# ArturKKK/graphcast-lite

Measured on AMD Instinct MI355X. Metric: training samples/sec (6h windows) + achieved HBM GB/s on mesh GCNConv, higher is better.
Workload: dtype f32

## Files before the change

graphcast-lite_amd/csrc/linear.hip:

```cpp
#include "common.h"
#include "mfma_io.h"
#include "x3.h"

namespace {

using namespace gcl::mfma_io;

#include "gemm_tile.h"

#define gcl_lin_sync() ((abl & 8) != 0)

constexpr int lin_min_waves(int NS, int KT) { return (NS <= 2 && KT <= 64) ? 3 : (NS <= 2 && KT <= 128) ? 2 : 1; }
constexpr bool lin_zpre(int NS, int EPI) { return EPI == 1 && NS >= 4; }

template <int NS, int EPI, int KT, bool VEC>
__global__ __launch_bounds__(256, lin_min_waves(NS, KT)) void linear_mfma_kernel(const float* __restrict__ X, int64_t ldx,
                                                          const float* __restrict__ in_slope,
                                                          const float* __restrict__ W, int32_t ldw, int32_t trans,
                                                          const float* __restrict__ bias, float* __restrict__ Y,
                                                          int64_t ldy, int64_t rows, int32_t K, int32_t N,
                                                          const float* __restrict__ Z, int64_t ldz,
                                                          const float* __restrict__ z_slope,
                                                          double* __restrict__ slope_part, int32_t akind,
                                                          int32_t abl) {
// ... 1152 lines not shown
  do {                                                                                                            \
    auto kern = gemm_tile_kernel<EPI, T_, MI_>;                                                                   \
    GCL_ENSURE_DYN_LDS(kern, gcl::kLdsBytes);                                                                     \
    hipLaunchKernelGGL(kern, dim3(g.grid), dim3(256), gt_lds(MI_), st, X, ldx, akind, slope, W, ldw, bias, Y, ldy, \
                       rows, K, N, Z, ldz, add, ldadd, slope_part, g.nt, g.total, g.per_xcd);                     \
  } while (0)
  if (trans) {
    if (g.mi == 1) GCL_GT(true, 1);
    else GCL_GT(true, 2);
  } else {
    if (g.mi == 1) GCL_GT(false, 1);
    else GCL_GT(false, 2);
  }
#undef GCL_GT
  GCL_CHECK_LAUNCH();
  if (nparts) *nparts = (int)g.grid;
  return GCL_OK;
}

}

extern "C" size_t gcl_colsum_ws_bytes(int64_t, int32_t);
extern "C" int gcl_colsum(const float*, int64_t, int64_t, int32_t, float*, int32_t, void*, size_t, gcl_stream_t);

static int check_act(const char* who, int act, const float* slope) {
  GCL_CHECK_ARG(act == GCL_ACT_NONE || act == GCL_ACT_PRELU || act == GCL_ACT_SILU, "%s: unknown activation %d", who, act);
  GCL_CHECK_ARG(act != GCL_ACT_PRELU || slope, "%s: GCL_ACT_PRELU needs the slope pointer", who);
  return GCL_OK;
}

extern "C" int gcl_dense_fwd(const float* x, int64_t ldx, int32_t act, const float* slope, const float* W, int64_t ldw,
                             const float* bias, const float* addend, int64_t ldadd, float* y, int64_t ldy,
                             int64_t rows, int32_t Fin, int32_t Fout, gcl_stream_t stream) {
  GCL_CHECK_ARG(x && W && y, "dense_fwd: null argument");
  GCL_CHECK_ARG(rows >= 0 && Fin >= 1 && Fout >= 1 && ldx >= Fin && ldy >= Fout && ldw >= Fin && (!addend || ldadd >= Fout),
                "dense_fwd: bad shape rows=%lld ldx=%lld ldy=%lld ldw=%lld", (long long)rows, (long long)ldx,
                (long long)ldy, (long long)ldw);
  if (int rc = check_act("dense_fwd", act, slope)) return rc;
  const bool vec_x = (Fin % 4 == 0) && (ldx % 4 == 0) && gcl::aligned16(x);
  if (!addend && ldw == Fin && !use_valu() && gcl::x3_linear_fwd_applicable(x, ldx, y, ldy, Fin, Fout, act))
    return gcl::x3_linear_fwd(x, ldx, act, act == GCL_ACT_PRELU ? slope : nullptr, W, bias, y, ldy, rows, Fin, Fout,
                              (hipStream_t)stream);
  if (!addend && ldw == Fin && (use_valu() || panel_fits(Fin, Fout, vec_x, false, (ldw % 4 == 0) && gcl::aligned16(W))))
    return launch_linear<EPI_BIAS>(x, ldx, act == GCL_ACT_PRELU ? slope : nullptr, W, Fin, 0, bias, y, ldy, rows, Fin,
                                   Fout, nullptr, 0, nullptr, nullptr, nullptr, (hipStream_t)stream, act);
  return launch_gemm<EPI_BIAS>(x, ldx, act, act == GCL_ACT_PRELU ? slope : nullptr, W, ldw, 0, bias, y, ldy, rows, Fin,
                               Fout, nullptr, 0, addend, ldadd, nullptr, nullptr, (hipStream_t)stream);
}

extern "C" int gcl_linear_fwd(const float* x, int64_t ldx, const float* in_slope, const float* W, const float* bias,
                              float* y, int64_t ldy, int64_t rows, int32_t Fin, int32_t Fout, gcl_stream_t stream) {
  return gcl_dense_fwd(x, ldx, in_slope ? GCL_ACT_PRELU : GCL_ACT_NONE, in_slope, W, Fin, bias, nullptr, 0, y, ldy, rows,
                       Fin, Fout, stream);
}

static size_t slope_parts_cap(int64_t rows, int32_t Fin) {
  const int64_t g = (int64_t)gt_geom(rows, Fin).grid;
  return (size_t)(g > 4096 ? g : 4096);
}

extern "C" size_t gcl_linear_bwd_ws_bytes(int64_t rows, int32_t Fin, int32_t Fout) {
  size_t nc = (size_t)(Fin + 31) / 32;
  if (nc > 4) nc = 4;
  const size_t FinP = nc * 32;
  size_t no = (size_t)(Fout + 31) / 32;
  no = no <= 2 ? no : no <= 4 ? 4 : 8;
  const size_t FoutP = no * 32;
  const size_t dw = (size_t)kDwBlocks * FoutP * (FinP + 1) * sizeof(float);
  const size_t sl = slope_parts_cap(rows, Fin) * sizeof(double);
  return dw + sl;
}

extern "C" int gcl_dense_bwd_dx(const float* dy, int64_t lddy, const float* W, int64_t ldw, const float* z, int64_t ldz,
                                int32_t act, const float* slope, float* d_slope, const float* addend, int64_t ldadd,
                                float* dx, int64_t lddx, int64_t rows, int32_t Fin, int32_t Fout, void* ws,
                                size_t ws_bytes, gcl_stream_t stream) {
  GCL_CHECK_ARG(dy && W && dx, "dense_bwd_dx: null argument");
  GCL_CHECK_ARG(lddy >= Fout && lddx >= Fin && ldw >= Fin && (!addend || ldadd >= Fin), "dense_bwd_dx: leading dimension too small");
  if (int rc = check_act("dense_bwd_dx", act, slope)) return rc;
  GCL_CHECK_ARG(act == GCL_ACT_NONE || (z && ldz >= Fin), "dense_bwd_dx: activation given without its pre-activation z");
  hipStream_t st = (hipStream_t)stream;
  const float* sl = act == GCL_ACT_PRELU ? slope : nullptr;
  double* slope_part = nullptr;
  if (sl && d_slope) {
    GCL_CHECK_ARG(ws && ws_bytes >= slope_parts_cap(rows, Fin) * sizeof(double) && gcl::aligned16(ws), "dense_bwd_dx: workspace too small");
    slope_part = (double*)ws;
  }
  int nparts = 0, rc;
  const float* zz = act == GCL_ACT_NONE ? nullptr : z;
  const bool vec_x = (Fout % 4 == 0) && (lddy % 4 == 0) && gcl::aligned16(dy);
  if (!addend && ldw == Fin && (use_valu() || panel_fits(Fout, Fin, vec_x, true, (ldw % 4 == 0) && gcl::aligned16(W))))
    rc = launch_linear<EPI_DX>(dy, lddy, nullptr, W, Fin, 1, nullptr, dx, lddx, rows, Fout, Fin, zz, ldz, sl, slope_part,
                               &nparts, st, act);
  else {
    const size_t off = (slope_parts_cap(rows, Fin) * sizeof(double) + 255) & ~(size_t)255;
    const size_t need = off + (size_t)Fin * Fout * sizeof(float);
    if (ws && ws_bytes >= need && gcl::aligned16(ws) && Fout % 4 == 0 && rows >= 4096) {
      float* Wt = reinterpret_cast<float*>(static_cast<char*>(ws) + off);
      hipLaunchKernelGGL(transpose_kernel, dim3((unsigned)gcl::cdiv(Fin, 32), (unsigned)gcl::cdiv(Fout, 32)), dim3(256), 0,
                         st, W, ldw, Wt, Fout, Fin);
      rc = launch_gemm<EPI_DX>(dy, lddy, act, sl, Wt, Fout, 0, nullptr, dx, lddx, rows, Fout, Fin, zz, ldz, addend,
                               ldadd, slope_part, &nparts, st);
    } else {
      rc = launch_gemm<EPI_DX>(dy, lddy, act, sl, W, ldw, 1, nullptr, dx, lddx, rows, Fout, Fin, zz, ldz, addend, ldadd,
                               slope_part, &nparts, st);
    }
// ... 351 lines not shown
```

graphcast-lite_amd/csrc/linear_x3.hip:

```cpp
#include "mfma_io.h"
#include "x3.h"

namespace {

typedef unsigned int u32x2 __attribute__((ext_vector_type(2)));

#ifndef GCL_X3_ST_AUX
#define GCL_X3_ST_AUX 2
#endif
__device__ __forceinline__ float4 ld_stream(const float4* p) {
#ifndef GCL_X3_LD_PLAIN
  typedef float lv4f __attribute__((ext_vector_type(4)));
  const lv4f v = __builtin_nontemporal_load(reinterpret_cast<const lv4f*>(p));
  return make_float4(v.x, v.y, v.z, v.w);
#else
  return *p;
#endif
}
using namespace gcl::mfma_io;
using namespace gcl::x3;

constexpr int kRowB = 144;
constexpr int kImgB = 32 * kRowB;
constexpr int kTileB = 3 * kImgB;
// ... 149 lines not shown
        const bf16x8 am = *reinterpret_cast<const bf16x8*>(ap + kImgB);
#pragma unroll
        for (int c = 0; c < NS; ++c) acc[c] = mfma_mid(acc[c], ah, am, wf[c][s][0], wf[c][s][1]);
      }
#pragma unroll
      for (int s = 0; s < NKS; ++s) {
        const bf16x8 ah = *reinterpret_cast<const bf16x8*>(Aw + fo + s * 32);
#pragma unroll
        for (int c = 0; c < NS; ++c) acc[c] = mfma_hi(acc[c], ah, wf[c][s][0]);
      }
    }

#ifdef GCL_STAMPS
    asm volatile("" ::"v"(acc[0][0]));
#endif
    X3_STAMP(4);
    const int64_t r0 = t * 128 + wave * 32;
    const int64_t nr64 = rows - r0;
    const int nr = nr64 < 0 ? 0 : (nr64 < 32 ? (int)nr64 : 32);
    constexpr int OS = NS * 32, LPO = OS / 4, RPP = 64 / LPO;
    float* Ot = reinterpret_cast<float*>(Aw);
#pragma unroll
    for (int s = 0; s < NS; ++s)
#pragma unroll
      for (int r = 0; r < 16; ++r) Ot[d_row(r, lane) * OS + s * 32 + (lane & 31)] = acc[s][r];
    const __amdgpu_buffer_rsrc_t ry = make_rsrc(Y + r0 * ldy, (nr > 0 && !(abl & 1)) ? ((int64_t)(nr - 1) * ldy + N) * 4 : 0);
    const int orow = lane / LPO, ocol = (lane % LPO) * 4;
#pragma unroll
    for (int p = 0; p < 32 / RPP; ++p) {
      const int i = p * RPP + orow;
      float4 v = *reinterpret_cast<const float4*>(Ot + i * OS + ocol);
      v.x += bq.x; v.y += bq.y; v.z += bq.z; v.w += bq.w;
      buf_st4<GCL_X3_ST_AUX>(ry, (ocol < N) ? (unsigned)((i * ldy + ocol) * 4) : kOOB, v);
    }
    X3_STAMP(5);
  }
#ifdef GCL_STAMPS
  if (lane == 0 && blockIdx.x < 1024)
    for (int i = 0; i < 8; ++i) x3_stamps[(blockIdx.x * 4 + wave) * 8 + i] = stamp_acc[i];
#endif
}

constexpr int kBRowB = 128;
constexpr int kImg64B = 64 * kBRowB;
__device__ __forceinline__ int swz(int r) { return (((r >> 1) & 1) << 2) | (((r >> 3) & 1) << 1) | ((r >> 2) & 1); }
__device__ __forceinline__ int sw_off(int r, int b) { return r * kBRowB + ((((b >> 4) ^ swz(r)) << 4) | (b & 15)); }

typedef short s16x4 __attribute__((ext_vector_type(4)));
__device__ __forceinline__ bf16x8 tr_frag(const unsigned char* base, int o0, int o1) {
  typedef __attribute__((address_space(3))) s16x4 lds_s16x4;
  const s16x4 a = __builtin_amdgcn_ds_read_tr16_b64_v4i16((lds_s16x4*)(base + o0));
  const s16x4 b = __builtin_amdgcn_ds_read_tr16_b64_v4i16((lds_s16x4*)(base + o1));
  return __builtin_shufflevector(a, b, 0, 1, 2, 3, 4, 5, 6, 7);
}

template <int NO>
__global__ __launch_bounds__(256, 2) void linear_x3_bwd_kernel(
    const float* __restrict__ dY, int64_t lddy, const float* __restrict__ W, const float* __restrict__ P,
    int64_t ldp, const float* __restrict__ in_slope, float* __restrict__ dX, int64_t lddx, int64_t rows, int32_t Fin,
    int32_t Fout, float* __restrict__ part_dw, float* __restrict__ part_db, float* __restrict__ part_cs,
    double* __restrict__ part_slope) {
  constexpr int FoP = NO * 32, FiP = 64, NKO = NO * 2, NT = NO * 2;
  extern __shared__ __align__(16) unsigned char smem8[];
  unsigned char* Yimg = smem8;
  unsigned char* Pimg = smem8 + 3 * kImg64B;
  float* Stg = reinterpret_cast<float*>(smem8 + 6 * kImg64B);
  const int tid = threadIdx.x, lane = tid & 63, wave = __builtin_amdgcn_readfirstlane(tid >> 6);
  const int li = lane & 31, h = lane >> 5;
  const int rg = wave & 1, sg = wave >> 1;
  const int so = wave % NO, sc = wave / NO;
  const bool has_tile = wave < NT;

  bf16x8 wtf[NKO][3];
  {
    float2 wv[8];
#pragma unroll
    for (int i = 0; i < 8; ++i) {
      const int idx = i * 256 + tid;
      const int c = idx & 63, o = (idx >> 6) * 2;
      wv[i].x = (c < Fin && o < Fout) ? W[(int64_t)o * Fin + c] : 0.f;
      wv[i].y = (c < Fin && o + 1 < Fout) ? W[(int64_t)(o + 1) * Fin + c] : 0.f;
    }
#pragma unroll
    for (int i = 0; i < 8; ++i) {
      const int idx = i * 256 + tid;
      const int c = idx & 63, o = (idx >> 6) * 2;
      const Pk3 p = split2(wv[i].x, wv[i].y);
      unsigned char* d = Yimg + sw_off(c, o * 2);
      *reinterpret_cast<unsigned*>(d) = p.h;
      *reinterpret_cast<unsigned*>(d + kImg64B) = p.m;
      *reinterpret_cast<unsigned*>(d + 2 * kImg64B) = p.l;
    }
    __syncthreads();
#pragma unroll
    for (int s = 0; s < NKO; ++s)
#pragma unroll
      for (int p = 0; p < 3; ++p)
        wtf[s][p] = *reinterpret_cast<const bf16x8*>(Yimg + p * kImg64B + sw_off(32 * sg + li, (16 * s + 8 * h) * 2));
    __syncthreads();
  }

  const bool act = in_slope != nullptr;
  const float slope = act ? *in_slope : 1.f;
  const int64_t ntiles = (rows + 63) / 64;

  const int rsub = lane >> 4, csub = lane & 15;
// ... 172 lines not shown
  return 0;
#endif
  static const int v = gcl::env_int("GCL_ABLATE", 0);
  return v;
}

}

#ifdef GCL_STAMPS
extern "C" int gcl_debug_read_stamps_x3(unsigned long long* host_out, int count) {
  GCL_CHECK_HIP(hipDeviceSynchronize());
  GCL_CHECK_HIP(hipMemcpyFromSymbol(host_out, HIP_SYMBOL(x3_stamps), sizeof(unsigned long long) * count));
  return GCL_OK;
}
#endif

namespace gcl {

bool x3_linear_fwd_applicable(const float* x, int64_t ldx, const float* y, int64_t ldy, int K, int N, int akind) {
  if (!env_int("GCL_X3", 1)) return false;
  if (K < 1 || K > 64 || N < 4 || N > 64 || (N & 3)) return false;
  if ((ldx & 3) || (ldy & 3) || !aligned16(x) || !aligned16(y)) return false;
  if (ldx * 4 * 35 >= ((int64_t)1 << 31) || ldy * 4 * 35 >= ((int64_t)1 << 31)) return false;
  return akind == kActNone || akind == kActPrelu || akind == kActSilu;
}

int x3_linear_fwd(const float* x, int64_t ldx, int akind, const float* slope, const float* W, const float* bias,
                  float* y, int64_t ldy, int64_t rows, int K, int N, hipStream_t st) {
  if (rows == 0) return GCL_OK;
  const int64_t ntiles = cdiv(rows, 128);
  const int grid = (int)(ntiles < 2 * kNumCU ? ntiles : 2 * kNumCU);
  const size_t lds = 4 * (size_t)kTileB;
#define GCL_X3F3(NS_, SILU_, NKS_)                                                                                \
  hipLaunchKernelGGL((linear_x3_fwd_kernel<NS_, SILU_, NKS_>), dim3(grid), dim3(256), lds, st, x, ldx, slope, akind, \
                     W, bias, y, ldy, rows, K, N, x3_ablate())
#define GCL_X3F(NS_, SILU_)           \
  do {                                \
    if (K <= 32) GCL_X3F3(NS_, SILU_, 2); \
    else GCL_X3F3(NS_, SILU_, 4);     \
  } while (0)
  if (akind == kActSilu) {
    if (N > 32) GCL_X3F(2, true);
    else GCL_X3F(1, true);
  } else {
    if (N > 32) GCL_X3F(2, false);
    else GCL_X3F(1, false);
  }
#undef GCL_X3F3
#undef GCL_X3F
  GCL_CHECK_LAUNCH();
  return GCL_OK;
}

bool x3_linear_bwd_applicable(const float* dy, int64_t lddy, const float* x, int64_t ldx, const float* dx, int64_t lddx,
                              int Fin, int Fout) {
  if (!env_int("GCL_X3", 1)) return false;
  if (Fin < 33 || Fin > 64 || (Fin & 3) || Fout < 1 || Fout > 64) return false;
  if (lddy < ((Fout + 3) & ~3) || (lddy & 3) || (ldx & 3) || (lddx & 3) || lddx < Fin) return false;
  if (!aligned16(dy) || !aligned16(x) || !aligned16(dx)) return false;
  return lddx * 4 * 70 < ((int64_t)1 << 31);
}

int x3_linear_bwd_blocks(int64_t rows) {
  const int64_t ntiles = cdiv(rows, 64);
  return (int)(ntiles < 2 * kNumCU ? ntiles : 2 * kNumCU);
}

int x3_linear_bwd(const float* dy, int64_t lddy, const float* W, const float* x, int64_t ldx, const float* in_slope,
                  float* dx, int64_t lddx, int64_t rows, int Fin, int Fout, float* part_dw, float* part_db,
                  float* part_cs, double* part_slope, hipStream_t st) {
  const int grid = x3_linear_bwd_blocks(rows);
  const size_t lds = 6 * (size_t)kImg64B + 64 * 64 * sizeof(float);
#define GCL_X3B(NO_)                                                                                              \
  do {                                                                                                            \
    auto kern = linear_x3_bwd_kernel<NO_>;                                                                        \
    GCL_ENSURE_DYN_LDS(kern, gcl::kLdsBytes);                                                                     \
    hipLaunchKernelGGL(kern, dim3(grid), dim3(256), lds, st, dy, lddy, W, x, ldx, in_slope, dx, lddx, rows, Fin, Fout, \
                       part_dw, part_db, part_cs, part_slope);                                                    \
  } while (0)
  if (Fout > 32) GCL_X3B(2);
  else GCL_X3B(1);
#undef GCL_X3B
  GCL_CHECK_LAUNCH();
  return GCL_OK;
}

}
```

graphcast-lite_amd/csrc/x3.h:

```cpp
#pragma once
#include "common.h"

namespace gcl {

bool x3_linear_fwd_applicable(const float* x, int64_t ldx, const float* y, int64_t ldy, int K, int N, int akind);
int x3_linear_fwd(const float* x, int64_t ldx, int akind, const float* slope, const float* W, const float* bias,
                  float* y, int64_t ldy, int64_t rows, int K, int N, hipStream_t st);

bool x3_linear_bwd_applicable(const float* dy, int64_t lddy, const float* x, int64_t ldx, const float* dx, int64_t lddx,
                              int Fin, int Fout);
int x3_linear_bwd_blocks(int64_t rows);
int x3_linear_bwd(const float* dy, int64_t lddy, const float* W, const float* x, int64_t ldx, const float* in_slope,
                  float* dx, int64_t lddx, int64_t rows, int Fin, int Fout, float* part_dw, float* part_db,
                  float* part_cs, double* part_slope, hipStream_t st);

}

#ifdef __HIPCC__
#include "mfma_io.h"

namespace gcl {
namespace x3 {

using mfma_io::f32x16;
typedef short bf16x8 __attribute__((ext_vector_type(8)));
typedef __bf16 bf16x2_t __attribute__((ext_vector_type(2)));
typedef float f32x2_t __attribute__((ext_vector_type(2)));

__device__ __forceinline__ unsigned pk_bf16(float a, float b) {
  return __builtin_bit_cast(unsigned, __builtin_convertvector(f32x2_t{a, b}, bf16x2_t));
}
struct Pk3 {
  unsigned h, m, l;
};
__device__ __forceinline__ Pk3 split2(float a, float b) {
  Pk3 p;
  p.h = pk_bf16(a, b);
  float ra = a - __uint_as_float(p.h << 16), rb = b - __uint_as_float(p.h & 0xffff0000u);
  p.m = pk_bf16(ra, rb);
  ra -= __uint_as_float(p.m << 16);
  rb -= __uint_as_float(p.m & 0xffff0000u);
  p.l = pk_bf16(ra, rb);
  return p;
}

__device__ __forceinline__ f32x16 mfma_lo(f32x16 acc, bf16x8 ah, bf16x8 am, bf16x8 al, bf16x8 bh, bf16x8 bm, bf16x8 bl) {
  acc = __builtin_amdgcn_mfma_f32_32x32x16_bf16(al, bh, acc, 0, 0, 0);
  acc = __builtin_amdgcn_mfma_f32_32x32x16_bf16(ah, bl, acc, 0, 0, 0);
  acc = __builtin_amdgcn_mfma_f32_32x32x16_bf16(am, bm, acc, 0, 0, 0);
  return acc;
}
__device__ __forceinline__ f32x16 mfma_mid(f32x16 acc, bf16x8 ah, bf16x8 am, bf16x8 bh, bf16x8 bm) {
  acc = __builtin_amdgcn_mfma_f32_32x32x16_bf16(am, bh, acc, 0, 0, 0);
  acc = __builtin_amdgcn_mfma_f32_32x32x16_bf16(ah, bm, acc, 0, 0, 0);
  return acc;
}
__device__ __forceinline__ f32x16 mfma_hi(f32x16 acc, bf16x8 ah, bf16x8 bh) {
  return __builtin_amdgcn_mfma_f32_32x32x16_bf16(ah, bh, acc, 0, 0, 0);
}

// ... 4 lines not shown
```

graphcast-lite_amd/functional.py:

```python
from typing import List, Optional

import os

import torch

from . import hip


def _grad_slot(p: Optional[torch.Tensor], needs: bool):
    if p is None or not needs:
        return None, False, True
    if p.grad is not None:
        return p.grad, True, True
    return torch.zeros_like(p), False, False


class _Grads:

    def __init__(self, params: List[Optional[torch.Tensor]], needs: List[bool]):
        self.dst, self.acc, self.ret_none = [], [], []
        for p, nd in zip(params, needs):
            d, a, r = _grad_slot(p, nd)
            self.dst.append(d)
            self.acc.append(a)
            self.ret_none.append(r)

    def out(self):
        return tuple(None if r else d for d, r in zip(self.dst, self.ret_none))


_ZERO = {}


def _token(like: torch.Tensor, shape):
    z = _ZERO.get(like.device)
    if z is None:
        if like.is_cuda and torch.cuda.is_current_stream_capturing():
            return like.new_zeros(()).expand(shape)
        with torch.inference_mode(False):
            z = _ZERO[like.device] = torch.zeros((), dtype=torch.float32, device=like.device)
    return z.expand(shape)


def _flat3(x: torch.Tensor):
    if x.dim() == 2:
        x = x.unsqueeze(0)
    if not x.is_contiguous():
        x = x.contiguous()
    return x


class MLPFn(torch.autograd.Function):
    @staticmethod
    def forward(ctx, x, owner, has_ln: bool, eps: float, *params):
        L = (len(params) - (2 if has_ln else 0) + 1) // 3
        shape = x.shape
        x2 = hip.rows2d(x.detach())
        zs = []
        cur, slope = x2, None
        for k in range(L):
            W, b = params[3 * k], params[3 * k + 1]
            z = hip.linear_fwd(cur, W.detach(), b.detach(), slope)
            zs.append(z)
            cur = z
            slope = params[3 * k + 2].detach() if k < L - 1 else None
        stats = None
        out = cur
        if has_ln:
            out, stats = hip.layernorm_fwd(cur, params[-2].detach(), params[-1].detach(), eps)
        ctx.owner, ctx.has_ln, ctx.L = owner, has_ln, L
        ctx.x2, ctx.zs, ctx.stats = x2, zs, stats
        ctx.params = params
        return out.view(shape[:-1] + (out.shape[-1],))

    @staticmethod
    def backward(ctx, dy):
        params, L = ctx.params, ctx.L
        needs = list(ctx.needs_input_grad[4:])
        G = _Grads(list(params), needs)
        dy2 = hip.rows2d(dy)
        zs = ctx.zs
        if ctx.has_ln:
            gi, bi = len(params) - 2, len(params) - 1
            dgam = G.dst[gi] if G.dst[gi] is not None else torch.zeros_like(params[gi])
            dbet = G.dst[bi] if G.dst[bi] is not None else torch.zeros_like(params[bi])
            dz = hip.layernorm_bwd(dy2, zs[-1], params[gi].detach(), ctx.stats, dgam, dbet, G.acc[gi] and G.acc[bi])
        else:
            dz = dy2
        dx = None
        for k in range(L - 1, -1, -1):
            W = params[3 * k].detach()
            inp = ctx.x2 if k == 0 else zs[k - 1]
            slope = None if k == 0 else params[3 * k - 1].detach()
            wi, bi = 3 * k, 3 * k + 1
            dW = G.dst[wi] if G.dst[wi] is not None else torch.zeros_like(params[wi])
            db = G.dst[bi]
            if k > 0:
                dz = hip.linear_bwd_all(dz, W, inp, slope, G.dst[3 * k - 1], dW, db, None, G.acc[wi], acc_db=G.acc[bi])
            elif ctx.needs_input_grad[0]:
                dx = hip.linear_bwd_all(dz, W, inp, None, None, dW, db, None, G.acc[wi], acc_db=G.acc[bi],
                                        act=hip.ACT_NONE)
            elif db is not None and G.acc[bi] != G.acc[wi]:
                hip.linear_bwd_dw(dz, inp, None, dW, None, G.acc[wi])
                hip.colsum(dz, db, G.acc[bi])
            else:
                hip.linear_bwd_dw(dz, inp, None, dW, db, G.acc[wi])
        if dx is not None:
            dx = dx.view(dy.shape[:-1] + (dx.shape[-1],))
        return (dx, None, None, None) + G.out()


_LN_COLSUM = os.environ.get("GCL_NO_LN_COLSUM", "0") in ("0", "")
_ROWS_OUT = os.environ.get("GCL_NO_ROWS_OUT", "0") in ("0", "")


def _row_skip() -> bool:
    return os.environ.get("GCL_NO_ROW_SKIP", "0") in ("0", "")

# ... 801 lines not shown
```

graphcast-lite_amd/hip.py:

```python
import ctypes as C
import os
from typing import Optional

import torch

_HERE = os.path.dirname(os.path.abspath(__file__))
LIB_PATH = os.environ.get("GCL_LIB") or os.path.join(_HERE, "libgcl_hip.so")

GRAPH_GCN, GRAPH_GAT, GRAPH_MEAN = 0, 1, 2

_lib = None

_i32, _i64, _f32, _vp, _sz = C.c_int32, C.c_int64, C.c_float, C.c_void_p, C.c_size_t

_SIGNATURES = {
    "gcl_version": (C.c_int, []),
    "gcl_last_error": (C.c_char_p, []),
    "gcl_graph_count_edges": (C.c_int, [_vp, _i64, _i32, _i32, C.POINTER(_i64)]),
    "gcl_graph_build_host": (C.c_int, [_vp, _i64, _i32, _i32] + [_vp] * 8),
    "gcl_graph_create": (C.c_int, [_vp, _i64, _i32, _i32, C.POINTER(_vp)]),
    "gcl_graph_destroy": (None, [_vp]),
    "gcl_graph_num_nodes": (_i32, [_vp]),
    "gcl_graph_num_edges": (_i64, [_vp]),
    "gcl_graph_max_in_degree": (_i32, [_vp]),
    "gcl_graph_export_edges": (C.c_int, [_vp, _vp]),
    "gcl_graph_eperm_device": (_vp, [_vp]),
    "gcl_graph_halo_info": (C.c_int, [_vp, _i32, _i32, _vp]),
    "gcl_linear_fwd": (C.c_int, [_vp, _i64, _vp, _vp, _vp, _vp, _i64, _i64, _i32, _i32, _vp]),
    "gcl_linear_bwd_dx": (C.c_int, [_vp, _i64, _vp, _vp, _i64, _vp, _vp, _vp, _i64, _i64, _i32, _i32, _vp, _sz, _vp]),
    "gcl_linear_bwd_dw": (C.c_int, [_vp, _i64, _vp, _i64, _vp, _vp, _vp, _i64, _i32, _i32, _i32, _vp, _sz, _vp]),
    "gcl_linear_bwd_ws_bytes": (_sz, [_i64, _i32, _i32]),
    "gcl_linear_bwd_all": (C.c_int, [_vp, _i64, _vp, _vp, _i64, _vp, _vp, _vp, _i64, _vp, _vp, _vp, _i64, _i32, _i32,
                                     _i32, _vp, _sz, _vp]),
    "gcl_linear_bwd_all_deferred": (C.c_int, [_vp, _i64, _vp, _vp, _i64, _vp, _vp, _vp, _i64, _vp, _vp, _vp, _i64, _i32,
                                              _i32, _i32, _vp, _sz, _vp, _vp]),
    "gcl_reduce_jobs": (C.c_int, [_vp, _i32, _vp]),
    "gcl_layernorm_bwd_deferred": (C.c_int, [_vp, _i64, _i64, _vp, _i32, _i32, _vp, _i64, _vp, _vp, _vp, _i64, _vp, _vp, _vp,
                                             _i32, _i64, _i32, _vp, _sz, _vp, _vp]),
    "gcl_colsum_deferred": (C.c_int, [_vp, _i64, _i64, _i32, _vp, _i32, _vp, _sz, _vp, _vp]),
    "gcl_colsum_split_deferred": (C.c_int, [_vp, _i64, _i64, _vp, _i64, _i64, _i32, _i32, _i32, _i32, _vp, _i32, _vp, _sz,
                                            _vp, _vp]),
    "gcl_linear_bwd_dw_deferred": (C.c_int, [_vp, _i64, _vp, _i64, _vp, _vp, _vp, _i64, _i32, _i32, _i32, _vp, _sz, _vp,
                                             _vp]),
    "gcl_dense_bwd_dw_deferred": (C.c_int, [_vp, _i64, _vp, _i64, _i32, _vp, _vp, _i64, _vp, _i64, _i32, _i32, _i32, _vp,
                                            C.c_size_t, _vp, _vp]),
    "gcl_linear_bwd_all_ws_bytes": (_sz, [_i64, _i32, _i32]),
    "gcl_aggregate": (C.c_int, [_vp, _i32, _vp, _i64, _i64, _vp, _vp, _i64, _i64, _i32, _i32, _vp]),
    "gcl_aggregate_present": (C.c_int, [_vp, _i32, _vp, _i64, _i64, _vp, _vp, _vp, _i64, _i64, _i32, _i32, _vp]),
    "gcl_aggregate_compact_ok": (C.c_int, [_vp, _i32, _i64, _i64, _i64, _i64, _i32, _i32]),
    "gcl_aggregate_compact": (C.c_int, [_vp, _i32, _vp, _i64, _i64, _vp, _vp, _i64, _i64, _vp, _i64, _i64, _i32, _i32, _vp]),
    "gcl_aggregate_heavy_launches": (_i64, []),
    "gcl_aggregate_split": (C.c_int, [_vp, _i32, _vp, _i64, _i64, _vp, _i64, _i64, _i32, _vp, _vp, _i64, _i64, _i32, _i32,
                                      _vp]),
    "gcl_gat_fwd": (C.c_int, [_vp, _vp, _i64, _i64, _vp, _vp, _vp, _vp, _vp, _vp, _vp, _i64, _i64, _i32, _i32, _i32, _vp]),
    "gcl_gat_bwd": (C.c_int, [_vp, _vp, _i64, _i64, _vp, _i64, _i64, _vp, _vp, _vp, _vp, _vp, _vp, _i64, _i64,
                              _vp, _vp, _vp, _i32, _i32, _i32, _i32, _vp, _sz, _vp]),
    "gcl_gat_bwd_ws_bytes": (_sz, [_i64, _i32, _i32, _i32, _i32]),
    "gcl_gat_fwd_tab": (C.c_int, [_vp, _vp, _i64, _i64, _vp, _vp, _vp, _vp, _vp, _vp, _vp, _vp, _i64, _i64, _i32, _i32, _i32, _vp]),
    "gcl_gat_bwd_tab": (C.c_int, [_vp, _vp, _i64, _i64, _vp, _i64, _i64, _vp, _vp, _vp, _vp, _vp, _vp, _vp, _i64, _i64,
                                  _vp, _vp, _vp, _i32, _i32, _i32, _i32, _vp, _sz, _vp]),
    "gcl_gat_tab_ok": (C.c_int, [_vp, _i64, _i32, _i32]),
    "gcl_gat_alpha_to_edge_order": (C.c_int, [_vp, _vp, _vp, _i32, _vp]),
    "gcl_gat_prune": (C.c_int, [_vp, _vp, _f32, _vp, C.POINTER(_i64), _vp, _sz, _vp]),
    "gcl_gat_prune_ws_bytes": (_sz, [_i64]),
    "gcl_layernorm_fwd": (C.c_int, [_vp, _i64, _vp, _vp, _f32, _vp, _i64, _vp, _i64, _i32, _vp]),
    "gcl_layernorm_bwd": (C.c_int, [_vp, _i64, _vp, _i64, _vp, _vp, _vp, _i64, _vp, _vp, _i32, _i64, _i32, _vp, _sz, _vp]),
    "gcl_layernorm_bwd_cs": (C.c_int, [_vp, _i64, _vp, _i64, _vp, _vp, _vp, _i64, _vp, _vp, _vp, _i32, _i64, _i32, _vp, _sz, _vp]),
    "gcl_layernorm_bwd_map": (C.c_int, [_vp, _i64, _i64, _vp, _i32, _vp, _i64, _vp, _vp, _vp, _i64, _vp, _vp, _vp, _i32, _i64,
                                        _i32, _vp, _sz, _vp]),
    "gcl_layernorm_fwd_map_skip": (C.c_int, [_vp, _i64, _vp, _vp, _f32, _vp, _i64, _i64, _vp, _i32, _vp, _i32, _vp, _i64, _i32,
                                             _vp]),
    "gcl_layernorm_bwd_map_skip": (C.c_int, [_vp, _i64, _i64, _vp, _i32, _vp, _i64, _vp, _vp, _vp, _i64, _vp, _vp, _vp, _i32,
                                             _i64, _i32, _vp, _sz, _vp]),
    "gcl_layernorm_bwd_ws_bytes": (_sz, [_i64, _i32]),
    "gcl_graphnorm_fwd": (C.c_int, [_vp, _i64, _i64, _vp, _vp, _f32, _vp, _i64, _i64, _vp, _i32, _i32, _i32, _vp, _sz, _vp]),
    "gcl_graphnorm_bwd": (C.c_int, [_vp, _i64, _i64, _vp, _i64, _i64, _vp, _vp, _f32, _vp, _i64, _i64, _vp, _vp,
                                    _i32, _i32, _i32, _i32, _vp, _sz, _vp]),
    "gcl_graphnorm_ws_bytes": (_sz, [_i32, _i32, _i32]),
    "gcl_colsum": (C.c_int, [_vp, _i64, _i64, _i32, _vp, _i32, _vp, _sz, _vp]),
    "gcl_colsum_ws_bytes": (_sz, [_i64, _i32]),
    "gcl_colsum_split": (C.c_int, [_vp, _i64, _i64, _vp, _i64, _i64, _i32, _i32, _i32, _i32, _vp, _i32, _vp, _sz, _vp]),
# ... 218 lines not shown
            self._exported[key] = t
        return t

    def __del__(self):
        try:
            if self._h:
                lib().gcl_graph_destroy(self._h)
                self._h = _vp()
        except Exception:
            pass


def build_csr_host(edge_index: torch.Tensor, num_nodes: int, kind: int):
    ei = edge_index.detach().to("cpu", torch.int64).contiguous()
    e_out = _i64(0)
    _check(lib().gcl_graph_count_edges(ei.data_ptr(), ei.shape[1], int(num_nodes), kind, C.byref(e_out)))
    Ep, n = e_out.value, int(num_nodes)
    i32 = lambda k: torch.zeros(max(k, 1), dtype=torch.int32)
    f32 = lambda k: torch.zeros(max(k, 1), dtype=torch.float32)
    out = dict(rowptr=i32(n + 1), col=i32(Ep), w=f32(Ep), eperm=i32(Ep), trowptr=i32(n + 1), tcol=i32(Ep),
               tw=f32(Ep), tslot=i32(Ep))
    _check(lib().gcl_graph_build_host(
        ei.data_ptr(), ei.shape[1], n, kind, out["rowptr"].data_ptr(), out["col"].data_ptr(), out["w"].data_ptr(),
        out["eperm"].data_ptr(), out["trowptr"].data_ptr(), out["tcol"].data_ptr(), out["tw"].data_ptr(),
        out["tslot"].data_ptr()))
    for k in ("col", "w", "eperm", "tcol", "tw", "tslot"):
        out[k] = out[k][:Ep]
    out["num_edges"] = Ep
    return out


def _ld(t: torch.Tensor) -> int:
    assert t.dim() == 2 and t.stride(1) == 1, "expected a [rows, F] view with unit channel stride"
    return t.stride(0) if t.shape[0] > 1 else max(t.stride(0), t.shape[1])


def _act_of(act, slope):
    return (ACT_PRELU if slope is not None else ACT_NONE) if act is None else int(act)


def linear_fwd(x, W, bias, in_slope, out=None, ld_out=None, act=None):
    rows, Fin = x.shape
    Fout = W.shape[0]
    if out is None:
        ld = ld_out or Fout
        out = torch.empty(rows, ld, dtype=torch.float32, device=x.device)[:, :Fout]
    if rows == 0:
        return out
    _check(lib().gcl_dense_fwd(_p(x), _ld(x), _act_of(act, in_slope), _p(in_slope), _p(W), W.stride(0), _p(bias), None, 0,
                               _p(out), _ld(out), rows, Fin, Fout, _stream()))
    return out


def linear_bwd_dx(dy, W, x, in_slope, d_in_slope, act=None):
    a = _act_of(act, in_slope)
    return dense_bwd_dx(dy, W, x if a != ACT_NONE else None, a, in_slope, d_in_slope)


def linear_bwd_dw(dy, x, in_slope, dW, db, accumulate: bool, act=None):
    dense_bwd_dw(dy, x, dW, db, accumulate, _act_of(act, in_slope), in_slope)


ACT_NONE, ACT_PRELU, ACT_SILU = 0, 1, 2


PROBE = None


def _probe_begin(kind, **info):
    return PROBE.begin(kind, **info) if PROBE is not None else None


def _probe_end(tok):
    if tok is not None:
        PROBE.end(tok)


def dense_fwd(x, W, bias, act=ACT_NONE, slope=None, addend=None, out=None):
    rows, Fin = x.shape
    Fout = W.shape[0]
    assert W.shape[1] == Fin and W.stride(1) == 1 and x.stride(1) == 1
    if out is None:
        out = torch.empty(rows, Fout, dtype=torch.float32, device=x.device)
    if rows == 0:
        return out
    tok = _probe_begin("dense_fwd", rows=rows, Fin=Fin, Fout=Fout)
    _check(lib().gcl_dense_fwd(_p(x), _ld(x), int(act), _p(slope), _p(W), W.stride(0), _p(bias), _p(addend),
                               _ld(addend) if addend is not None else 0, _p(out), _ld(out), rows, Fin, Fout, _stream()))
    _probe_end(tok)
    return out


def dense_bwd_dx(dy, W, z=None, act=ACT_NONE, slope=None, d_slope=None, addend=None, out=None):
    rows, Fout = dy.shape
    Fin = W.shape[1]
    assert W.shape[0] == Fout and W.stride(1) == 1
    if out is None:
        out = torch.empty(rows, Fin, dtype=torch.float32, device=dy.device)
    if rows == 0:
        return out
    nb = lib().gcl_linear_bwd_ws_bytes(rows, Fin, Fout)
    ws = workspace(nb, dy.device)
    _check(lib().gcl_dense_bwd_dx(_p(dy), _ld(dy), _p(W), W.stride(0), _p(z), _ld(z) if z is not None else 0, int(act),
                                  _p(slope), _p(d_slope), _p(addend), _ld(addend) if addend is not None else 0, _p(out),
                                  _ld(out), rows, Fin, Fout, ws.data_ptr(), ws.numel(), _stream()))
    return out
# ... 1169 lines not shown
```

include/gcl.h:

```cpp
#ifndef GCL_H
#define GCL_H

#include <stddef.h>
#include <stdint.h>

#ifdef __cplusplus
extern "C" {
#endif

#define GCL_VERSION 100

#define GCL_OK 0
#define GCL_EINVAL (-1)
#define GCL_EHIP (-2)
#define GCL_ENOMEM (-3)
#define GCL_EUNSUPPORTED (-4)

typedef struct gcl_graph gcl_graph_t;
typedef void* gcl_stream_t;

int gcl_version(void);
const char* gcl_last_error(void);

#define GCL_GRAPH_GCN 0
#define GCL_GRAPH_GAT 1
#define GCL_GRAPH_MEAN 2

int gcl_graph_count_edges(const int64_t* edge_index, int64_t E, int32_t n, int32_t kind, int64_t* e_out);

int gcl_graph_build_host(const int64_t* edge_index, int64_t E, int32_t n, int32_t kind,
                         int32_t* rowptr, int32_t* col, float* w, int32_t* eperm,
                         int32_t* trowptr, int32_t* tcol, float* tw, int32_t* tslot);

int gcl_graph_create(const int64_t* edge_index, int64_t E, int32_t n, int32_t kind, gcl_graph_t** out);
void gcl_graph_destroy(gcl_graph_t* g);
int32_t gcl_graph_num_nodes(const gcl_graph_t* g);
int64_t gcl_graph_num_edges(const gcl_graph_t* g);
int32_t gcl_graph_max_in_degree(const gcl_graph_t* g);
int gcl_graph_export_edges(const gcl_graph_t* g, int64_t* edge_index_out);
const int32_t* gcl_graph_eperm_device(const gcl_graph_t* g);
int gcl_graph_halo_info(const gcl_graph_t* g, int32_t transpose, int32_t T, int32_t* out4);

int gcl_linear_fwd(const float* x, int64_t ldx, const float* in_slope, const float* W ,
                   const float* bias , float* y, int64_t ldy, int64_t rows,
                   int32_t Fin, int32_t Fout, gcl_stream_t stream);

int gcl_linear_bwd_dx(const float* dy, int64_t lddy, const float* W, const float* x, int64_t ldx,
                      const float* in_slope, float* d_in_slope, float* dx, int64_t lddx,
                      int64_t rows, int32_t Fin, int32_t Fout, void* ws, size_t ws_bytes,
                      gcl_stream_t stream);
int gcl_linear_bwd_dw(const float* dy, int64_t lddy, const float* x, int64_t ldx,
                      const float* in_slope, float* dW, float* db, int64_t rows, int32_t Fin,
                      int32_t Fout, int32_t accumulate, void* ws, size_t ws_bytes,
                      gcl_stream_t stream);
size_t gcl_linear_bwd_ws_bytes(int64_t rows, int32_t Fin, int32_t Fout);
#define GCL_ACC_DW 1
#define GCL_ACC_DB 2
#define GCL_ACC_COLSUM 4
int gcl_linear_bwd_all(const float* dy, int64_t lddy, const float* W, const float* x, int64_t ldx,
                       const float* in_slope, float* d_in_slope, float* dx, int64_t lddx, float* dW,
                       float* db, float* colsum_dx, int64_t rows, int32_t Fin, int32_t Fout,
                       int32_t accumulate, void* ws, size_t ws_bytes, gcl_stream_t stream);
size_t gcl_linear_bwd_all_ws_bytes(int64_t rows, int32_t Fin, int32_t Fout);

typedef struct gcl_reduce_job {
  const float* part;
  int64_t pstride;
  struct {
    float* out;
    int32_t poff, count, pld, cols, ldo, acc;
  } seg[3];
  const double* spart;
  float* sout;
  int32_t nparts, ns;
} gcl_reduce_job;
int gcl_linear_bwd_all_deferred(const float* dy, int64_t lddy, const float* W, const float* x, int64_t ldx,
                                const float* in_slope, float* d_in_slope, float* dx, int64_t lddx, float* dW,
                                float* db, float* colsum_dx, int64_t rows, int32_t Fin, int32_t Fout,
                                int32_t accumulate, void* ws, size_t ws_bytes, gcl_stream_t stream,
                                gcl_reduce_job* job);
int gcl_reduce_jobs(const gcl_reduce_job* jobs, int32_t n, gcl_stream_t stream);
int gcl_layernorm_bwd_deferred(const float* dy, int64_t lddy, int64_t bsdy, const int32_t* pos, int32_t n_per,
                               int32_t skip, const float* x, int64_t ldx, const float* gamma, const float* stats,
                               float* dx, int64_t lddx, float* dgamma, float* dbeta, float* colsum_dx,
                               int32_t accumulate, int64_t rows, int32_t F, void* ws, size_t ws_bytes,
                               gcl_stream_t stream, gcl_reduce_job* job);
int gcl_colsum_deferred(const float* x, int64_t ldx, int64_t rows, int32_t F, float* out, int32_t accumulate, void* ws,
                        size_t ws_bytes, gcl_stream_t stream, gcl_reduce_job* job);
int gcl_colsum_split_deferred(const float* a, int64_t lda, int64_t bsa, const float* b, int64_t ldb, int64_t bsb,
                              int32_t head, int32_t n, int32_t B, int32_t F, float* out, int32_t accumulate, void* ws,
                              size_t ws_bytes, gcl_stream_t stream, gcl_reduce_job* job);
int gcl_linear_bwd_dw_deferred(const float* dy, int64_t lddy, const float* x, int64_t ldx, const float* in_slope,
                               float* dW, float* db, int64_t rows, int32_t Fin, int32_t Fout, int32_t accumulate,
                               void* ws, size_t ws_bytes, gcl_stream_t stream, gcl_reduce_job* job );
int gcl_dense_bwd_dw_deferred(const float* dy, int64_t lddy, const float* x, int64_t ldx, int32_t act,
                              const float* slope, float* dW, int64_t lddw, float* db, int64_t rows, int32_t Fin,
                              int32_t Fout, int32_t accumulate, void* ws, size_t ws_bytes, gcl_stream_t stream,
                              gcl_reduce_job* job );
// ... 369 lines not shown
```

Baseline: 26990.

## Fuse chained MLP linear layers into one persistent x3-MFMA forward kernel

Adds a fused forward kernel that runs 2-3 consecutive linear layers (with PReLU between them) per row tile. All layer weights stay resident in LDS as split bf16x3 images, and each layer's output is fed straight from registers and LDS into the next layer. The Python MLP forward picks the longest fusable run and falls back to per-layer linear_fwd otherwise. This removes separate kernel launches and the HBM re-read of intermediate activations. Every intermediate is still written out for backward, and the kernel uses one large-LDS block per CU, which may limit occupancy.

```diff
diff --git a/graphcast-lite_amd/csrc/linear.hip b/graphcast-lite_amd/csrc/linear.hip
--- a/graphcast-lite_amd/csrc/linear.hip
+++ b/graphcast-lite_amd/csrc/linear.hip
@@ -1228,6 +1228,31 @@
                               float* y, int64_t ldy, int64_t rows, int32_t Fin, int32_t Fout, gcl_stream_t stream) {
   return gcl_dense_fwd(x, ldx, in_slope ? GCL_ACT_PRELU : GCL_ACT_NONE, in_slope, W, Fin, bias, nullptr, 0, y, ldy, rows,
                        Fin, Fout, stream);
+}
+
+extern "C" int32_t gcl_mlp_fused_ok(int32_t L, const int32_t* widths, const int32_t* acts, const void* const* ptrs,
+                                    const int64_t* lds, int32_t nptr) {
+  if (gcl::env_int("GCL_NO_MLP_FUSED", 0) != 0 || use_valu()) return 0;
+  if (nptr < 0 || (nptr > 0 && (!ptrs || !lds))) return 0;
+  return gcl::x3_mlp_applicable(L, widths, acts, ptrs, lds, nptr) ? 1 : 0;
+}
+
+extern "C" int gcl_mlp_fwd(const float* x, int64_t ldx, int32_t L, const int32_t* widths, const float* const* W,
+                           const float* const* bias, const float* const* in_slope, float* const* y, const int64_t* ldy,
+                           int64_t rows, gcl_stream_t stream) {
+  GCL_CHECK_ARG(x && widths && W && bias && in_slope && y && ldy, "mlp_fwd: null argument");
+  GCL_CHECK_ARG(L >= 2 && L <= 3 && rows >= 0, "mlp_fwd: L = %d layers (2 or 3), rows = %lld", L, (long long)rows);
+  const void* ptrs[4] = {x, nullptr, nullptr, nullptr};
+  int64_t lds[4] = {ldx, 0, 0, 0};
+  int32_t acts[3];
+  for (int k = 0; k < L; ++k) {
+    GCL_CHECK_ARG(W[k] && y[k] && ldy[k] >= widths[k + 1], "mlp_fwd: layer %d: null argument or ldy too small", k);
+    ptrs[k + 1] = y[k], lds[k + 1] = ldy[k];
+    acts[k] = in_slope[k] ? GCL_ACT_PRELU : GCL_ACT_NONE;
+  }
+  GCL_CHECK_ARG(ldx >= widths[0], "mlp_fwd: ldx too small");
+  GCL_CHECK_ARG(gcl_mlp_fused_ok(L, widths, acts, ptrs, lds, L + 1), "mlp_fwd: the fused kernel does not take this chain");
+  return gcl::x3_mlp_fwd(x, ldx, L, widths, W, bias, in_slope, y, ldy, rows, (hipStream_t)stream);
 }
 
 static size_t slope_parts_cap(int64_t rows, int32_t Fin) {
diff --git a/graphcast-lite_amd/csrc/linear_x3.hip b/graphcast-lite_amd/csrc/linear_x3.hip
--- a/graphcast-lite_amd/csrc/linear_x3.hip
+++ b/graphcast-lite_amd/csrc/linear_x3.hip
@@ -225,6 +225,165 @@
   const s16x4 a = __builtin_amdgcn_ds_read_tr16_b64_v4i16((lds_s16x4*)(base + o0));
   const s16x4 b = __builtin_amdgcn_ds_read_tr16_b64_v4i16((lds_s16x4*)(base + o1));
   return __builtin_shufflevector(a, b, 0, 1, 2, 3, 4, 5, 6, 7);
+}
+
+constexpr int kMlpMaxL = 3;
+constexpr int kMlpWaves = 7;
+constexpr int kMlpWavesNarrow = 4;
+constexpr int kWLayerB = 3 * kImg64B;
+constexpr int kATileB = 3 * 32 * kBRowB;
+constexpr int kAImgB = 32 * kBRowB;
+struct MlpFwdArgs {
+  const float* W[kMlpMaxL];
+  const float* bias[kMlpMaxL];
+  const float* slope[kMlpMaxL];
+  float* Y[kMlpMaxL];
+  int64_t ldy[kMlpMaxL];
+  int32_t K[kMlpMaxL], N[kMlpMaxL];
+};
+
+template <int NS>
+__device__ __forceinline__ void mlp_x3_fwd_layer(float4 (&v8)[8], unsigned char* Aw, const unsigned char* Wimg, float pa,
+                                                 const float* __restrict__ bias, float* __restrict__ Y, int64_t ldy,
+                                                 int N, int64_t r0, int64_t rows, int lane) {
+  const int rsub = lane >> 4, csub = lane & 15;
+  float4 bq;
+  {
+    const int oc = (lane % (NS * 8)) * 4;
+    bq.x = (bias && oc < N) ? bias[oc] : 0.f;
+    bq.y = (bias && oc + 1 < N) ? bias[oc + 1] : 0.f;
+    bq.z = (bias && oc + 2 < N) ? bias[oc + 2] : 0.f;
+    bq.w = (bias && oc + 3 < N) ? bias[oc + 3] : 0.f;
+  }
+  __builtin_amdgcn_fence(__ATOMIC_ACQ_REL, "wavefront");
+#pragma unroll
+  for (int it = 0; it < 8; ++it) {
+    float4 v = v8[it];
+    const float mx = v.x * pa, my = v.y * pa, mz = v.z * pa, mw = v.w * pa;
+    v.x = v.x > 0.f ? v.x : mx; v.y = v.y > 0.f ? v.y : my;
+    v.z = v.z > 0.f ? v.z : mz; v.w = v.w > 0.f ? v.w : mw;
+    const Pk3 p01 = split2(v.x, v.y), p23 = split2(v.z, v.w);
+    unsigned char* d = Aw + sw_off(it * 4 + rsub, csub * 8);
+    *reinterpret_cast<u32x2*>(d) = u32x2{p01.h, p23.h};
+    *reinterpret_cast<u32x2*>(d + kAImgB) = u32x2{p01.m, p23.m};
+    *reinterpret_cast<u32x2*>(d + 2 * kAImgB) = u32x2{p01.l, p23.l};
+  }
+  const int li = lane & 31, h = lane >> 5;
+  int fo[4];
+#pragma unroll
+  for (int s = 0; s < 4; ++s) fo[s] = sw_off(li, (2 * s + h) * 16);
+  bf16x8 wf[NS][4][3];
+#pragma unroll
+  for (int t = 0; t < NS; ++t)
+#pragma unroll
+    for (int s = 0; s < 4; ++s)
+#pragma unroll
+      for (int p = 0; p < 3; ++p)
+        wf[t][s][p] = *reinterpret_cast<const bf16x8*>(Wimg + p * kImg64B + t * 32 * kBRowB + fo[s]);
+  f32x16 acc[NS];
+#pragma unroll
+  for (int s = 0; s < NS; ++s)
+#pragma unroll
+    for (int r = 0; r < 16; ++r) acc[s][r] = 0.f;
+#pragma unroll
+  for (int s = 0; s < 4; ++s) {
+    const unsigned char* ap = Aw + fo[s];
+    const bf16x8 ah = *reinterpret_cast<const bf16x8*>(ap);
+    const bf16x8 am = *reinterpret_cast<const bf16x8*>(ap + kAImgB);
+    const bf16x8 al = *reinterpret_cast<const bf16x8*>(ap + 2 * kAImgB);
+#pragma unroll
+    for (int c = 0; c < NS; ++c) acc[c] = mfma_lo(acc[c], ah, am, al, wf[c][s][0], wf[c][s][1], wf[c][s][2]);
+  }
+#pragma unroll
+  for (int s = 0; s < 4; ++s) {
+    const unsigned char* ap = Aw + fo[s];
+    const bf16x8 ah = *reinterpret_cast<const bf16x8*>(ap);
+    const bf16x8 am = *reinterpret_cast<const bf16x8*>(ap + kAImgB);
+#pragma unroll
+    for (int c = 0; c < NS; ++c) acc[c] = mfma_mid(acc[c], ah, am, wf[c][s][0], wf[c][s][1]);
+  }
+#pragma unroll
+  for (int s = 0; s < 4; ++s) {
+    const bf16x8 ah = *reinterpret_cast<const bf16x8*>(Aw + fo[s]);
+#pragma unroll
+    for (int c = 0; c < NS; ++c) acc[c] = mfma_hi(acc[c], ah, wf[c][s][0]);
+  }
+  const int64_t nr64 = rows - r0;
+  const int nr = nr64 < 0 ? 0 : (nr64 < 32 ? (int)nr64 : 32);
+  constexpr int OS = NS * 32, LPO = OS / 4, RPP = 64 / LPO;
+  float* Ot = reinterpret_cast<float*>(Aw);
+#pragma unroll
+  for (int s = 0; s < NS; ++s)
+#pragma unroll
+    for (int r = 0; r < 16; ++r) Ot[d_row(r, lane) * OS + s * 32 + (lane & 31)] = acc[s][r];
+  const __amdgpu_buffer_rsrc_t ry = make_rsrc(Y + r0 * ldy, nr > 0 ? ((int64_t)(nr - 1) * ldy + N) * 4 : 0);
+  const int orow = lane / LPO, ocol = (lane % LPO) * 4;
+#pragma unroll
+  for (int p = 0; p < 32 / RPP; ++p) {
+    const int i = p * RPP + orow;
+    float4 v = *reinterpret_cast<const float4*>(Ot + i * OS + ocol);
+    v.x += bq.x; v.y += bq.y; v.z += bq.z; v.w += bq.w;
+    buf_st4<GCL_X3_ST_AUX>(ry, (ocol < N) ? (unsigned)((i * ldy + ocol) * 4) : kOOB, v);
+    if (NS == 2) v8[p] = v;
+  }
+}
+
+template <int L, int NSL, int NW>
+__global__ __launch_bounds__(NW * 64, 1) void mlp_x3_fwd_kernel(const float* __restrict__ X, int64_t ldx, int64_t rows,
+                                                               const MlpFwdArgs a) {
+  constexpr int NT = NW * 64, TR = NW * 32;
+  extern __shared__ __align__(16) unsigned char smem8[];
+  const int tid = threadIdx.x, lane = tid & 63, wave = __builtin_amdgcn_readfirstlane(tid >> 6);
+  unsigned char* Aw = smem8 + L * kWLayerB + wave * kATileB;
+
+#pragma unroll
+  for (int l = 0; l < L; ++l) {
+    const float* __restrict__ W = a.W[l];
+    const int K = a.K[l], N = a.N[l];
+    for (int idx = tid; idx < 64 * 32; idx += NT) {
+      const int j = idx >> 5, k = (idx & 31) * 2;
+      const bool okj = j < N;
+      const float w0 = (okj && k < K) ? W[(int64_t)j * K + k] : 0.f;
+      const float w1 = (okj && k + 1 < K) ? W[(int64_t)j * K + k + 1] : 0.f;
+      const Pk3 p = split2(w0, w1);
+      unsigned char* d = smem8 + l * kWLayerB + sw_off(j, k * 2);
+      *reinterpret_cast<unsigned*>(d) = p.h;
+      *reinterpret_cast<unsigned*>(d + kImg64B) = p.m;
+      *reinterpret_cast<unsigned*>(d + 2 * kImg64B) = p.l;
+    }
+  }
+  __syncthreads();
+
+  float pa[L];
+#pragma unroll
+  for (int l = 0; l < L; ++l) pa[l] = a.slope[l] ? *a.slope[l] : 1.f;
+
+  const int rsub = lane >> 4, csub = lane & 15;
+  const bool cok = csub * 4 < a.K[0];
+  float4 pre[8], v8[8];
+  auto issue = [&](int64_t tile) {
+    const int64_t r0 = tile * TR + wave * 32;
+#pragma unroll
+    for (int it = 0; it < 8; ++it) {
+      const int64_t row = r0 + it * 4 + rsub;
+      const float4* p = (cok && row < rows) ? reinterpret_cast<const float4*>(X + row * ldx + csub * 4) : zero4;
+      pre[it] = ld_stream(p);
+    }
+  };
+
+  const int64_t ntiles = (rows + TR - 1) / TR;
+  issue(blockIdx.x);
+  for (int64_t t = blockIdx.x; t < ntiles; t += gridDim.x) {
+    const int64_t r0 = t * TR + wave * 32;
+#pragma unroll
+    for (int it = 0; it < 8; ++it) v8[it] = pre[it];
+    issue(t + gridDim.x);
+#pragma unroll
+    for (int l = 0; l < L - 1; ++l)
+      mlp_x3_fwd_layer<2>(v8, Aw, smem8 + l * kWLayerB, pa[l], a.bias[l], a.Y[l], a.ldy[l], a.N[l], r0, rows, lane);
+    mlp_x3_fwd_layer<NSL>(v8, Aw, smem8 + (L - 1) * kWLayerB, pa[L - 1], a.bias[L - 1], a.Y[L - 1], a.ldy[L - 1], a.N[L - 1], r0,
+                          rows, lane);
+  }
 }
 
 template <int NO>
@@ -503,6 +662,52 @@
   return GCL_OK;
 }
 
+bool x3_mlp_applicable(int L, const int* widths, const int* acts, const void* const* ptrs, const int64_t* lds, int nptr) {
+  if (!env_int("GCL_X3", 1)) return false;
+  if (L < 2 || L > kMlpMaxL || !widths || !acts) return false;
+  for (int k = 0; k < L; ++k) {
+    if (widths[k] < 36 || widths[k] > 64 || (widths[k] & 3)) return false;
+    if (acts[k] != kActNone && acts[k] != kActPrelu) return false;
+  }
+  if (widths[L] < 4 || widths[L] > 64 || (widths[L] & 3)) return false;
+  for (int i = 0; i < nptr; ++i)
+    if (!ptrs[i] || !aligned16(ptrs[i]) || (lds[i] & 3) || lds[i] * 4 * 70 >= ((int64_t)1 << 31)) return false;
+  return true;
+}
+
+int x3_mlp_fwd(const float* x, int64_t ldx, int L, const int* widths, const float* const* W, const float* const* bias,
+               const float* const* slope, float* const* y, const int64_t* ldy, int64_t rows, hipStream_t st) {
+  if (rows == 0) return GCL_OK;
+  MlpFwdArgs a;
+  memset(&a, 0, sizeof(a));
+  for (int k = 0; k < L; ++k) {
+    a.W[k] = W[k], a.bias[k] = bias[k], a.slope[k] = slope[k], a.Y[k] = y[k], a.ldy[k] = ldy[k];
+    a.K[k] = widths[k], a.N[k] = widths[k + 1];
+  }
+  const bool wide = widths[L] > 32;
+  const int nw = wide ? kMlpWaves : kMlpWavesNarrow;
+  const int64_t ntiles = cdiv(rows, nw * 32);
+  const int grid = (int)(ntiles < kNumCU ? ntiles : kNumCU);
+  const size_t lds = (size_t)L * kWLayerB + nw * (size_t)kATileB;
+#define GCL_MLPF(L_, NSL_)                                                               \
+  do {                                                                                   \
+    constexpr int NW_ = NSL_ == 2 ? kMlpWaves : kMlpWavesNarrow;                        \
+    auto kern = mlp_x3_fwd_kernel<L_, NSL_, NW_>;                                        \
+    GCL_ENSURE_DYN_LDS(kern, gcl::kLdsBytes);                                            \
+    hipLaunchKernelGGL(kern, dim3(grid), dim3(NW_ * 64), lds, st, x, ldx, rows, a);      \
+  } while (0)
+  if (L == 2) {
+    if (wide) GCL_MLPF(2, 2);
+    else GCL_MLPF(2, 1);
+  } else {
+    if (wide) GCL_MLPF(3, 2);
+    else GCL_MLPF(3, 1);
+  }
+#undef GCL_MLPF
+  GCL_CHECK_LAUNCH();
+  return GCL_OK;
+}
+
 bool x3_linear_bwd_applicable(const float* dy, int64_t lddy, const float* x, int64_t ldx, const float* dx, int64_t lddx,
                               int Fin, int Fout) {
   if (!env_int("GCL_X3", 1)) return false;
diff --git a/graphcast-lite_amd/csrc/x3.h b/graphcast-lite_amd/csrc/x3.h
--- a/graphcast-lite_amd/csrc/x3.h
+++ b/graphcast-lite_amd/csrc/x3.h
@@ -6,6 +6,10 @@
 bool x3_linear_fwd_applicable(const float* x, int64_t ldx, const float* y, int64_t ldy, int K, int N, int akind);
 int x3_linear_fwd(const float* x, int64_t ldx, int akind, const float* slope, const float* W, const float* bias,
                   float* y, int64_t ldy, int64_t rows, int K, int N, hipStream_t st);
+
+bool x3_mlp_applicable(int L, const int* widths, const int* acts, const void* const* ptrs, const int64_t* lds, int nptr);
+int x3_mlp_fwd(const float* x, int64_t ldx, int L, const int* widths, const float* const* W, const float* const* bias,
+               const float* const* slope, float* const* y, const int64_t* ldy, int64_t rows, hipStream_t st);
 
 bool x3_linear_bwd_applicable(const float* dy, int64_t lddy, const float* x, int64_t ldx, const float* dx, int64_t lddx,
                               int Fin, int Fout);
diff --git a/graphcast-lite_amd/functional.py b/graphcast-lite_amd/functional.py
--- a/graphcast-lite_amd/functional.py
+++ b/graphcast-lite_amd/functional.py
@@ -50,6 +50,13 @@
     return x
 
 
+def _mlp_run_ok(x2, Ws, slopes) -> bool:
+    if x2.shape[0] == 0 or not all(W.is_contiguous() for W in Ws):
+        return False
+    widths = [Ws[0].shape[1]] + [W.shape[0] for W in Ws]
+    return hip.mlp_fused_ok(widths, [hip.ACT_NONE if s is None else hip.ACT_PRELU for s in slopes], (x2,))
+
+
 class MLPFn(torch.autograd.Function):
     @staticmethod
     def forward(ctx, x, owner, has_ln: bool, eps: float, *params):
@@ -57,13 +64,19 @@
         shape = x.shape
         x2 = hip.rows2d(x.detach())
         zs = []
-        cur, slope = x2, None
-        for k in range(L):
-            W, b = params[3 * k], params[3 * k + 1]
-            z = hip.linear_fwd(cur, W.detach(), b.detach(), slope)
-            zs.append(z)
-            cur = z
-            slope = params[3 * k + 2].detach() if k < L - 1 else None
+        cur = x2
+        Ws = [params[3 * k].detach() for k in range(L)]
+        bs = [params[3 * k + 1].detach() for k in range(L)]
+        slopes = [None] + [params[3 * k + 2].detach() for k in range(L - 1)]
+        k = 0
+        while k < L:
+            n = next((n for n in range(min(3, L - k), 1, -1) if _mlp_run_ok(cur, Ws[k:k + n], slopes[k:k + n])), 1)
+            if n > 1:
+                zs += hip.mlp_fwd(cur, Ws[k:k + n], bs[k:k + n], slopes[k:k + n])
+            else:
+                zs.append(hip.linear_fwd(cur, Ws[k], bs[k], slopes[k]))
+            cur = zs[-1]
+            k += n
         stats = None
         out = cur
         if has_ln:
diff --git a/graphcast-lite_amd/hip.py b/graphcast-lite_amd/hip.py
--- a/graphcast-lite_amd/hip.py
+++ b/graphcast-lite_amd/hip.py
@@ -27,6 +27,8 @@
     "gcl_graph_eperm_device": (_vp, [_vp]),
     "gcl_graph_halo_info": (C.c_int, [_vp, _i32, _i32, _vp]),
     "gcl_linear_fwd": (C.c_int, [_vp, _i64, _vp, _vp, _vp, _vp, _i64, _i64, _i32, _i32, _vp]),
+    "gcl_mlp_fused_ok": (_i32, [_i32, _vp, _vp, _vp, _vp, _i32]),
+    "gcl_mlp_fwd": (C.c_int, [_vp, _i64, _i32, _vp, _vp, _vp, _vp, _vp, _vp, _i64, _vp]),
     "gcl_linear_bwd_dx": (C.c_int, [_vp, _i64, _vp, _vp, _i64, _vp, _vp, _vp, _i64, _i64, _i32, _i32, _vp, _sz, _vp]),
     "gcl_linear_bwd_dw": (C.c_int, [_vp, _i64, _vp, _i64, _vp, _vp, _vp, _i64, _i32, _i32, _i32, _vp, _sz, _vp]),
     "gcl_linear_bwd_ws_bytes": (_sz, [_i64, _i32, _i32]),
@@ -351,6 +353,29 @@
     return out
 
 
+def mlp_fused_ok(widths, acts, tensors=()) -> bool:
+    L = len(widths) - 1
+    n = len(tensors)
+    return bool(lib().gcl_mlp_fused_ok(L, (_i32 * (L + 1))(*widths), (_i32 * L)(*[int(a) for a in acts]),
+                                       (_vp * max(n, 1))(*[_p(t) for t in tensors]),
+                                       (_i64 * max(n, 1))(*[_ld(t) for t in tensors]), n))
+
+
+def mlp_fwd(x, Ws, biases, in_slopes):
+    L = len(Ws)
+    rows = x.shape[0]
+    widths = [x.shape[1]] + [W.shape[0] for W in Ws]
+    for k, W in enumerate(Ws):
+        assert tuple(W.shape) == (widths[k + 1], widths[k]) and W.is_contiguous(), "mlp_fwd: W_k must be a dense [Fout, Fin]"
+    zs = [torch.empty(rows, w, dtype=torch.float32, device=x.device) for w in widths[1:]]
+    if rows == 0:
+        return zs
+    arr = lambda ts: (_vp * L)(*[_p(t) for t in ts])
+    _check(lib().gcl_mlp_fwd(_p(x), _ld(x), L, (_i32 * (L + 1))(*widths), arr(Ws), arr(biases), arr(in_slopes), arr(zs),
+                             (_i64 * L)(*[_ld(z) for z in zs]), rows, _stream()))
+    return zs
+
+
 def linear_bwd_dx(dy, W, x, in_slope, d_in_slope, act=None):
     a = _act_of(act, in_slope)
     return dense_bwd_dx(dy, W, x if a != ACT_NONE else None, a, in_slope, d_in_slope)
diff --git a/include/gcl.h b/include/gcl.h
--- a/include/gcl.h
+++ b/include/gcl.h
@@ -44,6 +44,12 @@
 int gcl_linear_fwd(const float* x, int64_t ldx, const float* in_slope, const float* W ,
                    const float* bias , float* y, int64_t ldy, int64_t rows,
                    int32_t Fin, int32_t Fout, gcl_stream_t stream);
+
+int32_t gcl_mlp_fused_ok(int32_t L, const int32_t* widths, const int32_t* acts, const void* const* ptrs,
+                         const int64_t* lds, int32_t nptr);
+int gcl_mlp_fwd(const float* x, int64_t ldx, int32_t L, const int32_t* widths, const float* const* W,
+                const float* const* bias, const float* const* in_slope, float* const* y, const int64_t* ldy,
+                int64_t rows, gcl_stream_t stream);
 
 int gcl_linear_bwd_dx(const float* dy, int64_t lddy, const float* W, const float* x, int64_t ldx,
                       const float* in_slope, float* d_in_slope, float* dx, int64_t lddx,
```

New measurement: 27250, median of 6. Within noise of the previous version (+1.0%).
